# lvjiahui/DRT

Measured on AMD Instinct MI355X. Metric: M camera-rays/s (forward+backward) on 50k-tri mesh, 72 views, higher is better.
Workload: dtype f32 traversal + f64 shading/gradients; 1 GPU; horse_vh.ply x4 (1 midpoint subdivision) = 50248 tris / 25126 verts, 72 turntable views, 1024x1024 rays/view, LBVH rebuilt every step, forward+ray_loss+backward+all-reduce+SGD; targets=horse_scan.ply, mode=dropin, hip_graph=False, outputs_recycled=True, ray_binding=True, views_per_gpu=72, views_per_call=72

## Files before the change

### drt_amd/csrc/drt_api.hip

```cpp
#include "drt_scene.h"

static thread_local char g_err[512] = "";
int fail(int code, const char* fmt, ...) {
    va_list ap;
    va_start(ap, fmt);
    vsnprintf(g_err, sizeof(g_err), fmt, ap);
    va_end(ap);
    return code;
}

int ensure_slow_stack(drt_scene* s, hipStream_t st) {
    if (s->slow_stack) return DRT_OK;
    hipStreamCaptureStatus cap = hipStreamCaptureStatusNone;
    if (hipStreamIsCapturing(st, &cap) == hipSuccess && cap != hipStreamCaptureStatusNone)
        return fail(DRT_E_INVALID, "the first silhouette / closest-point / intersect query of a scene allocates its overflow area and cannot run inside a "
                                   "stream capture: issue one such call eagerly before capturing");
    int blocks = s->grid_trace;
    if (blocks < 4 * s->n_cu) blocks = 4 * s->n_cu;
    if (blocks < kRedoGrid) blocks = kRedoGrid;
    HIP_TRY(hipMalloc(&s->slow_stack, sizeof(int32_t) * (size_t)blocks * kTraceBlock * kStackSlowDev));
    return DRT_OK;
}

static int g_det = -1;
// ... 80 lines not shown
}

int drt_create(int device, drt_scene_t** out) {
    if (!out) return fail(DRT_E_INVALID, "out is null");
    int count = 0;
    HIP_TRY(hipGetDeviceCount(&count));
    if (device < 0 || device >= count) return fail(DRT_E_INVALID, "device %d out of range (%d visible)", device, count);
    HIP_TRY(hipSetDevice(device));
    drt_scene* s = new (std::nothrow) drt_scene();
    if (!s) return fail(DRT_E_NOMEM, "host allocation failed");
    s->device = device;
    hipError_t e = hipMalloc(&s->params, sizeof(BuildParams));
    if (e == hipSuccess) e = hipMalloc(&s->scratch, sizeof(unsigned long long) * 8);
    if (e == hipSuccess) e = hipMalloc(&s->bounds_acc, sizeof(uint32_t) * 12);
    if (e == hipSuccess) {
        const uint32_t init[12] = {0xFF800000u, 0xFF800000u, 0xFF800000u, 0x007FFFFFu, 0x007FFFFFu, 0x007FFFFFu,
                                   0xFF800000u, 0xFF800000u, 0xFF800000u, 0x007FFFFFu, 0x007FFFFFu, 0x007FFFFFu};
        e = hipMemcpy(s->bounds_acc, init, sizeof(init), hipMemcpyHostToDevice);
    }
    if (e == hipSuccess) e = hipMalloc(&s->vcount, sizeof(unsigned) * 4);
    if (e == hipSuccess) e = hipMemset(s->vcount, 0, sizeof(unsigned) * 4);
    if (e == hipSuccess) e = hipMalloc(&s->seg_counts, sizeof(unsigned) * drt_scene::kMaxSeg);
    if (e == hipSuccess) e = hipEventCreateWithFlags(&s->fork_ev, hipEventDisableTiming);
    if (e == hipSuccess) e = hipStreamCreateWithFlags(&s->build_stream, hipStreamNonBlocking);
    if (e == hipSuccess) e = hipEventCreateWithFlags(&s->prefill_fork, hipEventDisableTiming);
    if (e == hipSuccess) e = hipEventCreateWithFlags(&s->prefill_done, hipEventDisableTiming);
    if (e == hipSuccess) e = hipEventCreateWithFlags(&s->prefill_done_cap, hipEventDisableTiming);
    if (e == hipSuccess) e = hipEventCreateWithFlags(&s->build_fork, hipEventDisableTiming);
    if (e == hipSuccess) e = hipEventCreateWithFlags(&s->build_done, hipEventDisableTiming);
    if (const char* ev = getenv("DRT_ASYNC_BUILD")) s->async_build = atoi(ev) != 0;
    if (const char* ev = getenv("DRT_CULL_DIRECT")) s->cull_direct = atoi(ev) != 0;
    if (const char* ev = getenv("DRT_CULL_PARK")) s->cull_park = atoi(ev) != 0;
    if (const char* ev = getenv("DRT_CULL_DIRECT_MIN_LOG2")) { const int v = atoi(ev); if (v >= 0 && v <= 40) s->cull_direct_min_rays = (int64_t)1 << v; }
    if (const char* ev = getenv("DRT_TREE")) { const int v = atoi(ev); if (v >= 0 && v <= 2) s->tree_mode = v; }
    if (const char* ev = getenv("DRT_REBUILD_EVERY")) { const int v = atoi(ev); if (v >= 1) s->rebuild_every = v; }
    if (const char* ev = getenv("DRT_STREAMS")) { const int v = atoi(ev); if (v >= 1 && v <= drt_scene::kMaxSub) s->n_sub = v; }
    if (const char* ev = getenv("DRT_RASTER")) s->use_raster = atoi(ev) != 0;
    if (const char* ev = getenv("DRT_RASTER_DEAL")) s->raster_deal = atoi(ev) != 0;
    if (const char* ev = getenv("DRT_RASTER_DEAL_MIN_RUNS")) { const long long v = atoll(ev); if (v >= 0) s->raster_deal_min_runs = v; }
    if (const char* ev = getenv("DRT_RASTER_DEAL_FIXED")) { const int v = atoi(ev); if (v >= 1 && v <= 65536) s->raster_deal_fixed = (uint32_t)v; }
    if (const char* ev = getenv("DRT_HIT_SEED")) s->hit_seed = atoi(ev) != 0;
    if (const char* ev = getenv("DRT_ARM_FINISH_BESIDE")) s->arm_finish_beside = atoi(ev) != 0;
    if (const char* ev = getenv("DRT_SEED_TILED")) s->seed_tiled = atoi(ev) != 0;
    if (const char* ev = getenv("DRT_GRID_CANARY")) s->grid_canary = atoi(ev) != 0;
    if (const char* ev = getenv("DRT_FILL_OVERLAP")) s->fill_overlap = atoi(ev) != 0;
    if (const char* ev = getenv("DRT_FILL_AFTER_SHADE1")) s->fill_after_shade1 = atoi(ev) != 0;
    if (const char* ev = getenv("DRT_SUB_PER_STREAM")) { const int v = atoi(ev); if (v >= 1 && v <= 16) s->sub_per_stream = v; }
    if (const char* ev = getenv("DRT_MIN_SUB_LOG2")) { const int v = atoi(ev); if (v >= 12 && v <= 30) s->min_sub_rays = (int64_t)1 << v; }
    for (int k = 0; k < s->n_sub && e == hipSuccess; ++k) {
        drt_scene::Sub& w = s->sub[k];
        e = hipStreamCreateWithFlags(&w.stream, hipStreamNonBlocking);
        if (e == hipSuccess) e = hipEventCreateWithFlags(&w.done, hipEventDisableTiming);
        if (e == hipSuccess) e = hipEventCreateWithFlags(&w.tail, hipEventDisableTiming);
        if (e == hipSuccess) e = hipEventCreateWithFlags(&w.fill_fork, hipEventDisableTiming);
        if (e == hipSuccess) e = hipEventCreateWithFlags(&w.fill_join, hipEventDisableTiming);
        if (e == hipSuccess) e = hipMalloc(&w.qcount, sizeof(unsigned) * kQCount);
        if (e == hipSuccess) e = hipMalloc(&w.slow_stack, sizeof(int32_t) * (size_t)kRedoGrid * kTraceBlock * kStackSlowDev);
    }
    if (e == hipSuccess) {
        hipDeviceProp_t prop;
        if (hipGetDeviceProperties(&prop, device) == hipSuccess && prop.multiProcessorCount > 0) s->n_cu = prop.multiProcessorCount;
        int per_cu;
        per_cu = query_blocks_per_cu();
        s->grid_trace = s->n_cu * per_cu;
        if (s->grid_trace > kTraceGridMax) s->grid_trace = kTraceGridMax;
        per_cu = pipeline_blocks_per_cu();
        s->grid_path = s->n_cu * per_cu;
        if (s->grid_path * 2 > kTraceGridMax) s->grid_path = kTraceGridMax / 2;
        per_cu = mega_blocks_per_cu();
        s->grid_mega = s->n_cu * per_cu;
        if (const char* e = getenv("DRT_MEGA_BPC")) { const int v = atoi(e); if (v >= 1 && v <= 8) s->grid_mega = v * s->n_cu; }
        if (const char* e = getenv("DRT_MEGA_MAX_LOG2")) { const int v = atoi(e); s->mega_max_rays = v <= 0 ? 0 : (v <= 31 ? (int64_t)1 << v : (int64_t)1 << 31); }
        if (const char* e = getenv("DRT_SHADE_MIN")) { const int v = atoi(e); if (v >= 1 && v <= 64) s->shade_min = v; }
        if (const char* e = getenv("DRT_MEGA_REFILL_MIN")) { const int v = atoi(e); if (v >= 1 && v <= 64) s->mega_refill_min = v; }
        if (const char* e = getenv("DRT_TRACE_BPC")) { const int v = atoi(e); if (v >= 1 && v * s->n_cu * 2 <= kTraceGridMax) s->grid_path = v * s->n_cu; }
        if (const char* e = getenv("DRT_INNER_MIN")) { const int v = atoi(e); if (v >= 1 && v <= 64) s->inner_min = v; }
        if (const char* e = getenv("DRT_REFILL_MIN")) { const int v = atoi(e); if (v >= 1 && v <= 64) s->refill_min = v; }
        if (const char* e = getenv("DRT_CHUNK_LOG2")) { const int v = atoi(e); if (v >= 16 && v <= 30) s->chunk_rays = (int64_t)1 << v; }
    }
    if (e != hipSuccess) {
        drt_destroy(s);
        return fail(DRT_E_HIP, "hipMalloc: %s", hipGetErrorString(e));
    }
    *out = s;
    return DRT_OK;
}

void drt_destroy(drt_scene_t* s) {
    if (!s) return;
    (void)hipSetDevice(s->device);
    if (s->build_stream) (void)hipStreamSynchronize(s->build_stream);
    scene_free_mesh(s);
    if (s->build_fork) (void)hipEventDestroy(s->build_fork);
    if (s->build_done) (void)hipEventDestroy(s->build_done);
    if (s->build_stream) (void)hipStreamDestroy(s->build_stream);
    (void)hipFree(s->params);
    (void)hipFree(s->slow_stack);
    (void)hipFree(s->scratch); (void)hipFree(s->bounds_acc); (void)hipFree(s->seg_counts);
    (void)hipFree(s->b1_list); (void)hipFree(s->b1_redo); (void)hipFree(s->b1_count);
    for (int j = 0; j < drt_scene::kMaxSub; ++j) {
        drt_scene::Sub& w = s->sub[j];
        for (int k = 0; k < 3; ++k) { (void)hipFree(w.q_idx[k]); (void)hipFree(w.q_ray[k]); (void)hipFree(w.q_face[k]); }
        (void)hipFree(w.tmp_face1); (void)hipFree(w.tmp_face2); (void)hipFree(w.qcount); (void)hipFree(w.slow_stack); (void)hipFree(w.redo);
        (void)hipFree(w.zbuf); (void)hipFree(w.zmask); (void)hipFree(w.vmodel); (void)hipFree(w.big); (void)hipFree(w.big_count); (void)hipFree(w.gen_list); (void)hipFree(w.ray64);
        (void)hipFree(w.deal.table);
        if (w.done) (void)hipEventDestroy(w.done);
        if (w.fill_fork) (void)hipEventDestroy(w.fill_fork);
        if (w.fill_join) (void)hipEventDestroy(w.fill_join);
        if (w.tail) (void)hipEventDestroy(w.tail);
        if (w.stream) (void)hipStreamDestroy(w.stream);
    }
    image_views_free(s);
    image_loss_free(s);
    paths_free(s);
    (void)hipFree(s->vcount);
    (void)hipFree(s->vh_list);
    if (s->fork_ev) (void)hipEventDestroy(s->fork_ev);
    if (s->prefill_fork) (void)hipEventDestroy(s->prefill_fork);
    if (s->prefill_done) (void)hipEventDestroy(s->prefill_done);
    if (s->prefill_done_cap) (void)hipEventDestroy(s->prefill_done_cap);
    for (auto& e : s->prof_ev) (void)hipEventDestroy(e);
    (void)hipFree(s->prof_counts);
    delete s;
}

int drt_profile_enable(drt_scene_t* s, int on) {
    CHECK_SCENE(s);
    if (on && s->prof_ev.empty()) {
        s->prof_ev.resize(8192);
        s->prof_stage.resize(4096);
        for (auto& e : s->prof_ev) HIP_TRY(hipEventCreate(&e));
        HIP_TRY(hipMalloc(&s->prof_counts, sizeof(unsigned long long) * (kProfStages + 12)));
        HIP_TRY(hipMemset(s->prof_counts, 0, sizeof(unsigned long long) * (kProfStages + 12)));
    }
    s->prof_on = on != 0;
    s->prof_stats = on == 2;
    s->prof_serial = on == 3;
    return DRT_OK;
}

int drt_profile_select(drt_scene_t* s, uint32_t stage_mask) {
// ... 77 lines not shown
```

### drt_amd/csrc/drt_pipeline.hip

```cpp
#include "drt_device.h"
#include "drt_trace_kernel.h"
#include "drt_pathsink.h"


struct Ray64 {
    double* o;
    double* d;
};
struct Pipe {
    RayList r0, r1, r2;
    unsigned* count;
    unsigned* valid;
    int32_t* redo;
};




__device__ __forceinline__ void write_dead(int64_t i, double* out_ori, double* out_dir, uint8_t* mask, int32_t* face2) {
    const d3 z{0.0, 0.0, 0.0};
    store_d3(out_ori, i, z);
    store_d3(out_dir, i, z);
    mask[3 * i] = 0; mask[3 * i + 1] = 0; mask[3 * i + 2] = 0;
    face2[i] = -1;
// ... 1098 lines not shown
        w.tmp_face1 = w.tmp_face2 = nullptr; w.fused_cap = 0;
        HIP_TRY(hipMalloc(&w.tmp_face1, sizeof(int32_t) * n));
        HIP_TRY(hipMalloc(&w.tmp_face2, sizeof(int32_t) * n));
        w.fused_cap = n;
    }
    return DRT_OK;
}

static Pipe pipe_of(const drt_scene* s, const drt_scene::Sub& w) {
    return Pipe{RayList{w.q_idx[0], w.q_ray[0], w.q_face[0]}, RayList{w.q_idx[1], w.q_ray[1], w.q_face[1]},
                RayList{w.q_idx[2], w.q_ray[2], w.q_face[2]}, w.qcount, s->vcount, w.redo};
}

struct Plan { int64_t size; int count; int streams; };
static Plan plan_call(const drt_scene* s, int64_t n_rays, int tile_w, int tile_h) {
    int64_t unit = 256;
    if (tile_w >= 64 && tile_w % 64 == 0) unit = 4 * (int64_t)tile_w;
    if (unit > 256 && tile_h >= 4 && tile_h % 4 == 0 && n_rays % ((int64_t)tile_w * tile_h) == 0) unit = (int64_t)tile_w * tile_h;
    int64_t count = (n_rays + s->chunk_rays - 1) / s->chunk_rays;
    const int64_t by_min = n_rays / s->min_sub_rays;
    const int64_t most = (int64_t)s->n_sub * s->sub_per_stream;
    const int64_t want = by_min < most ? by_min : most;
    if (want > count) count = want;
    if (count < 1) count = 1;
    int64_t size = (n_rays + count - 1) / count;
    size = (size + unit - 1) / unit * unit;
    count = (n_rays + size - 1) / size;
    Plan pl;
    pl.size = size; pl.count = (int)count; pl.streams = count < s->n_sub ? (int)count : s->n_sub;
    if (s->prof_serial) pl.streams = 1;
    return pl;
}

__global__ void k_store_models(const ViewModel* __restrict__ work, ViewModel* __restrict__ cache, int n) {
    const int v = blockIdx.x * blockDim.x + threadIdx.x;
    if (v >= n) return;
    ViewModel m = work[v];
    m.all = (m.ok && m.all) ? 1 : 0;
    m.ok = m.all;
    cache[v] = m;
}

static bool raster_on(const drt_scene* s, int64_t n, int tile_w, int tile_h) {
    if (!s->use_raster || s->n_faces <= 0 || tile_w < 64 || tile_w % 64 != 0 || tile_h < 4 || tile_h % 4 != 0) return false;
    const int64_t image = (int64_t)tile_w * tile_h;
    return n > 0 && n % image == 0 && n / image <= 65535;
}

constexpr int kIntPreOri = 1 << 16, kIntPreDir = 1 << 17, kIntPreMask = 1 << 18, kIntMask = kIntPreOri | kIntPreDir | kIntPreMask;
extern "C++" {
template <bool FUSED>
static int launch_chunk(drt_scene* s, drt_scene::Sub& w, hipStream_t st, const PathCtx& pc, const Pipe& p, const double* o, const double* d, const uint8_t* valid,
                        int64_t n, double* out_ori, double* out_dir, uint8_t* mask, int32_t* face1, int32_t* face2, int tile_w, int tile_h,
                        int grid_mode, ViewModel* grid_cache ,
                        hipStream_t aux , int64_t chunk_base, int32_t* valid_idx,
                        bool* n_finished ,
                        int32_t* seed2 = nullptr ) {
    if (n_finished) *n_finished = false;
    const bool sparse_faces = (grid_mode & DRT_GRID_SPARSE_FACES) != 0;
    const bool pre_ori = (grid_mode & kIntPreOri) != 0, pre_dir = (grid_mode & kIntPreDir) != 0, pre_mask = (grid_mode & kIntPreMask) != 0;
    const bool all_verified = (grid_mode & DRT_GRID_ALL_VERIFIED) != 0 && (grid_mode & 3) == DRT_GRID_TRUST && grid_cache;
    grid_mode &= 3;
    const int gs = 8 * s->n_cu;
    if (tile_w < 64 || tile_w % 64 != 0 || n % (4 * (int64_t)tile_w) != 0) tile_w = 0;
    RasterIn rz{nullptr, 0, nullptr, nullptr, nullptr, 0, 0, 0, 0};
    const bool mega = s->mega_max_rays > 0 && n <= s->mega_max_rays && n_finished != nullptr;
    const Ray64 r64 = !mega ? Ray64{nullptr, nullptr} : (FUSED ? Ray64{w.ray64, w.ray64 + 3 * n} : Ray64{out_ori, out_dir});
    bool late_fill = false;
    hipStream_t fs = s->prof_serial ? st : s->build_stream;
    {
        hipStreamCaptureStatus cs = hipStreamCaptureStatusNone;
        if (fs != st && hipStreamIsCapturing(st, &cs) == hipSuccess && cs != hipStreamCaptureStatusNone) fs = aux ? aux : st;
    }
    const int64_t image = (int64_t)tile_w * tile_h;
    if (raster_on(s, n, tile_w, tile_h)) {
        const int n_views = (int)(n / image);
        int rc = ensure_raster(s, w, n, n_views, st);
        if (rc) return rc;
        if (!grid_cache) grid_mode = DRT_GRID_NONE;
        if (!FUSED && grid_mode == DRT_GRID_TRUST) {
            late_fill = s->fill_overlap;
            if (!late_fill) {
                StageTimer t(s, st, kStageFill);
                if (!pre_ori) (void)hipMemsetAsync(out_ori, 0, sizeof(double) * 3 * n, st);
                if (!pre_dir) (void)hipMemsetAsync(out_dir, 0, sizeof(double) * 3 * n, st);
                if (!pre_mask) (void)hipMemsetAsync(mask, 0, 3 * n, st);
            }
            if (!sparse_faces) { (void)hipMemsetAsync(face1, 0xFF, sizeof(int32_t) * n, st); (void)hipMemsetAsync(face2, 0xFF, sizeof(int32_t) * n, st); }
        }
        if (late_fill && mega) {
            if (fs != st && aux) fs = aux;
            if (fs != st) { HIP_TRY(hipEventRecord(w.fill_fork, st)); HIP_TRY(hipStreamWaitEvent(fs, w.fill_fork, 0)); }
            { StageTimer tf(s, fs, kStageFill);
              if (!pre_ori) (void)hipMemsetAsync(out_ori, 0, sizeof(double) * 3 * n, fs);
              if (!pre_dir) (void)hipMemsetAsync(out_dir, 0, sizeof(double) * 3 * n, fs);
              if (!pre_mask) (void)hipMemsetAsync(mask, 0, 3 * n, fs); }
            if (fs != st) HIP_TRY(hipEventRecord(w.fill_join, fs));
        }
        StageTimer t(s, st, kStageRaster);
        rc = launch_raster(s, w, st, o, d, n_views, tile_w, tile_h, grid_mode == DRT_GRID_TRUST ? grid_cache : nullptr);
        if (rc) return rc;
        rz = RasterIn{w.vmodel, grid_mode, w.zbuf, w.zmask, w.gen_list, tile_w, tile_h, all_verified ? 1 : 0, all_verified ? 1 : 0};
    }
    const bool pre_any = pre_ori || pre_dir || pre_mask;
    if (pre_any && !late_fill) HIP_TRY(hipStreamWaitEvent(st, s->prefill_done, 0));
    const bool tree_late = all_verified && rz.views != nullptr;
    if (!tree_late) { int rc = wait_build(s, st); if (rc) return rc; }
    const bool direct = s->cull_direct && rz.views && grid_mode == DRT_GRID_TRUST && !mega && n >= s->cull_direct_min_rays;
    const bool park = !FUSED && !mega && rz.views && grid_mode == DRT_GRID_TRUST && pre_ori && pre_dir && pre_mask && s->cull_park;
    const Ray64 r64p = park ? Ray64{out_ori, out_dir} : r64;
    if (park) HIP_TRY(hipStreamWaitEvent(st, s->prefill_done, 0));
    {
        int64_t* rc = s->route_counts;
        rc[kRouteTotal] += 1;
        rc[kRouteRaster] += rz.views != nullptr;
        rc[kRouteTrust] += rz.views && grid_mode == DRT_GRID_TRUST;
        rc[kRouteDirect] += direct;
        rc[kRoutePark] += park;
        rc[kRouteLateFill] += late_fill;
        rc[kRouteTreeLate] += tree_late;
        rc[kRouteMega] += mega;
    }
    { StageTimer t(s, st, kStageCull);
      const unsigned n_patches = (unsigned)((n + kPathBlock - 1) / kPathBlock);
      if (rz.views && grid_mode == DRT_GRID_TRUST) {
          uint32_t* list = reinterpret_cast<uint32_t*>(p.redo);
          k_patch_list<<<(n_patches + kPathBlock - 1) / kPathBlock, kPathBlock, 0, st>>>(n_patches, tile_w, rz, list, p.count + 7);
          static const int cull_per_cu = cull_blocks_per_cu();
          const unsigned few = (unsigned)(kCullFewPerCu * s->n_cu), long_list = few * (unsigned)(kCullRun * kCullLongRuns);
          k_cull_listed<FUSED><<<cull_per_cu * s->n_cu, kPathBlock, 0, st>>>(list, p.count + 7, pc.tc.nodes, pc.tc.n_tris, o, d, valid, n, out_ori, out_dir, mask, face1, face2, p, tile_w, rz,
                                                          pc, direct, late_fill, park ? Ray64{out_ori, out_dir} : Ray64{nullptr, nullptr}, few, long_list);
      } else {
          k_cull<FUSED><<<n_patches, kPathBlock, 0, st>>>(pc.tc.nodes, pc.tc.n_tris, o, d, valid, n, out_ori, out_dir, mask, face1, face2, p, tile_w, rz,
                                                          pre_ori && pre_dir && pre_mask && sparse_faces);
      } }
    auto issue_late_fills = [&]() -> int {
        if (fs != st) { HIP_TRY(hipEventRecord(w.fill_fork, st)); HIP_TRY(hipStreamWaitEvent(fs, w.fill_fork, 0)); }
        { StageTimer tf(s, fs, kStageFill);
          if (!pre_ori) (void)hipMemsetAsync(out_ori, 0, sizeof(double) * 3 * n, fs);
          if (!pre_dir) (void)hipMemsetAsync(out_dir, 0, sizeof(double) * 3 * n, fs);
          if (!pre_mask) (void)hipMemsetAsync(mask, 0, 3 * n, fs); }
        if (fs != st) HIP_TRY(hipEventRecord(w.fill_join, fs));
        return DRT_OK;
    };
    const bool fills_after_shade1 = s->fill_after_shade1 && fs != st;
    if (late_fill && !mega && !fills_after_shade1) { int rc = issue_late_fills(); if (rc) return rc; }
    if (rz.views && grid_mode == DRT_GRID_ESTABLISH)
        k_store_models<<<(int)(n / ((int64_t)tile_w * tile_h) + 63) / 64, 64, 0, st>>>(w.vmodel, grid_cache, (int)(n / ((int64_t)tile_w * tile_h)));
    { StageTimer t(s, st, kStageTrace1);
      if (rz.views && all_verified) {
      } else if (rz.views) {
          const TraceOut out{p.r0.face, nullptr, nullptr, w.gen_list};
          launch_trace_list(kTraceClosestListed, s->grid_path, st, pc.tc, p.r0.ray, p.count + 3, out, p.redo, p.count + 4, p.count + 16, s->refill_min, s->inner_min, s->prof_stats ? s->prof_counts + kProfStages + 4 * 0 : nullptr);
      } else {
          launch_trace_list(kTraceClosest, s->grid_path, st, pc.tc, p.r0.ray, p.count + 0, TraceOut{p.r0.face, nullptr, nullptr, nullptr}, p.redo, p.count + 4, p.count + 16, s->refill_min, s->inner_min, s->prof_stats ? s->prof_counts + kProfStages + 4 * 0 : nullptr);
      } }
    if (mega) {
        if (late_fill && fs != st) HIP_TRY(hipStreamWaitEvent(st, w.fill_join, 0));
        if (pre_any) HIP_TRY(hipStreamWaitEvent(st, s->prefill_done, 0));
    }
    {
      StageTimer t(s, st, kStageShade1);
// ... 138 lines not shown
    for (int k = 0; k < pl.streams; ++k) { int rc = ensure_queues(s->sub[k], pl.size, false); if (rc) return rc; }
    HIP_TRY(hipMemsetAsync(s->vcount, 0, sizeof(unsigned), st));
    const bool segmented = d_valid_idx != nullptr && pl.count >= 2 && pl.count <= drt_scene::kMaxSeg;
    if (segmented) HIP_TRY(hipMemsetAsync(s->seg_counts, 0, sizeof(unsigned) * pl.count, st));
    s->segs = drt_scene::Segs{};
    grid_mode &= ~kIntMask;
    hipStreamCaptureStatus cap = hipStreamCaptureStatusNone;
    (void)hipStreamIsCapturing(st, &cap);
    if (arm.loss && (cap != hipStreamCaptureStatusNone || (s->mega_max_rays > 0 && n_rays - (pl.count - 1) * pl.size <= s->mega_max_rays)))
        arm = drt_scene::LossArm{};
    if (s->n_prefill && (cap == hipStreamCaptureStatusNone || (s->clean.rows && s->clean.captured))) {
        int matched = 0;
        for (int k = 0; k < s->n_prefill; ++k) {
            const drt_scene::Prefill& f = s->prefill[k];
            const int before = grid_mode;
            if (f.ptr == d_out_ori && f.bytes == (int64_t)sizeof(double) * 3 * n_rays) grid_mode |= kIntPreOri;
            if (f.ptr == d_out_dir && f.bytes == (int64_t)sizeof(double) * 3 * n_rays) grid_mode |= kIntPreDir;
            if (f.ptr == d_mask && f.bytes == 3 * n_rays) grid_mode |= kIntPreMask;
            matched += grid_mode != before;
        }
        if (matched != s->n_prefill && cap == hipStreamCaptureStatusNone) HIP_TRY(hipStreamWaitEvent(st, s->prefill_done, 0));
        s->n_prefill = 0;
    }
    bool clean_late = s->clean.rows != nullptr && (grid_mode & 3) == DRT_GRID_TRUST && d_grid_cache != nullptr;
    for (int j = 0; j < pl.count && clean_late; ++j) {
        const int64_t b = j * pl.size, n = n_rays - b < pl.size ? n_rays - b : pl.size;
        clean_late = raster_on(s, n, tile_w, tile_h);
    }
    int rc = DRT_OK;
    if (s->clean.rows && !clean_late) { rc = flush_clean(s, st); if (rc) return rc; }
    rc = fork_streams(s, st, pl.streams);
    if (rc) return rc;
    if (s->clean.rows) { rc = flush_clean(s, st); if (rc) return rc; }
    bool finish_moved = false;
    for (int j = 0; j < pl.count; ++j) {
        drt_scene::Sub& w = s->sub[j % pl.streams];
        const int64_t b = j * pl.size;
        const int64_t n = n_rays - b < pl.size ? n_rays - b : pl.size;
        const PathCtx pc = sub_ctx(s, w, d_verts, ior_int, ior_ext);
        Pipe p = pipe_of(s, w);
        int32_t* vlist = d_valid_idx;
        if (segmented) { p.valid = s->seg_counts + j; vlist = d_valid_idx + b; }
        HIP_TRY(hipMemsetAsync(w.qcount, 0, kQCount * sizeof(unsigned), w.stream));
        bool finished = false;
        rc = launch_chunk<false>(s, w, w.stream, pc, p, d_origin + 3 * b, d_dir + 3 * b, nullptr, n, d_out_ori + 3 * b, d_out_dir + 3 * b,
                                 d_mask + 3 * b, d_face1 + b, d_face2 + b, tile_w, tile_h, grid_mode, sub_cache(d_grid_cache, b, tile_w, tile_h),
                                 st, b, vlist, &finished, seed2 ? seed2 + b : nullptr);
        if (rc) return rc;
        if (!finished) {
            hipStream_t fin = w.stream;
            if (arm.loss && s->arm_finish_beside && !s->prof_serial && j + pl.streams >= pl.count) {
                HIP_TRY(hipEventRecord(w.tail, w.stream));
                HIP_TRY(hipStreamWaitEvent(st, w.tail, 0));
                fin = st;
                finish_moved = true;
            }
            StageTimer t(s, fin, kStageFinish);
            k_finish<<<8 * s->n_cu, kPathBlock, 0, fin>>>(d_out_ori + 3 * b, d_out_dir + 3 * b, d_mask + 3 * b, d_face2 + b, p, b, vlist);
        }
        if (arm.loss) {
            if (finished) return fail(DRT_E_INVALID, "armed loss: a sub-batch took the one-kernel path");
            StageTimer t(s, w.stream, kStageBackward);
            DET_LAUNCH(k_loss_bwd_armed, DRT_BWD_BPC * s->n_cu, 256, w.stream, pc, d_origin + 3 * b, d_dir + 3 * b, arm.screen_pixel + 3 * b, arm.valid + b,
                                                                 d_face1 + b, d_face2 + b, p, arm.loss, arm.grad_verts);
        }
        if (s->prof_on) k_prof_counts<<<1, 64, 0, w.stream>>>(w.qcount, (unsigned long long)n, s->prof_counts, 0, raster_on(s, n, tile_w, tile_h), finished);
    }
    rc = join_streams(s, st, pl.streams);
    if (rc) return rc;
    if (segmented) {
        for (int j = 1; j < pl.count; ++j)
            k_join_lists<<<2 * s->n_cu, 256, 0, st>>>(d_valid_idx, s->seg_counts, j, (int64_t)j * pl.size, j + 1 == pl.count, s->vcount, d_n_valid);
        if (cap == hipStreamCaptureStatusNone && !finish_moved) s->segs = drt_scene::Segs{d_valid_idx, pl.count, 0};
    } else if (d_n_valid) {
        k_store_count<<<1, 64, 0, st>>>(s->vcount, d_n_valid);
    }
    if (s->prof_on) s->prof_stream = st;
    HIP_TRY(hipGetLastError());
    s->loss_taken = arm.loss != nullptr;
    return DRT_OK;
// ... 232 lines not shown
    HIP_TRY(hipGetLastError());
    return DRT_OK;
}

int drt_scale_rows3(double* d_x, const int32_t* d_list, const uint32_t* d_n_list, const double* d_scale, void* stream) {
    if (!d_x || !d_list || !d_n_list || !d_scale) return fail(DRT_E_INVALID, "null pointer argument");
    k_scale_rows3<<<1024, 256, 0, (hipStream_t)stream>>>(d_x, d_list, d_n_list, d_scale);
    HIP_TRY(hipGetLastError());
    return DRT_OK;
}

int drt_render_ray_loss_fused(drt_scene_t* s, const double* d_verts, const double* d_origin, const double* d_dir,
                              const double* d_screen_pixel, const uint8_t* d_valid, int64_t n_rays, double ior_int,
                              double ior_ext, double* d_loss, double* d_grad_verts, int64_t* d_n_valid, int tile_w, int tile_h,
                              int grid_mode, void* d_grid_cache, void* stream) {
    CHECK_BUILT(s);
    if (n_rays < 0 || n_rays > INT32_MAX) return fail(DRT_E_INVALID, "ray count out of range");
    if (n_rays == 0) return DRT_OK;
    if (!d_verts || !d_origin || !d_dir || !d_screen_pixel || !d_valid || !d_loss || !d_grad_verts) return fail(DRT_E_INVALID, "null pointer argument");
    hipStream_t st = (hipStream_t)stream;
    int32_t* const seed2 = take_seed(s, n_rays);
    (void)take_loss_arm(s, -1);
    const Plan pl = plan_call(s, n_rays, tile_w, tile_h);
    for (int k = 0; k < pl.streams; ++k) { int rc = ensure_queues(s->sub[k], pl.size, true, s->mega_max_rays > 0 && pl.size <= s->mega_max_rays); if (rc) return rc; }
    hipStreamCaptureStatus cap = hipStreamCaptureStatusNone;
    (void)hipStreamIsCapturing(st, &cap);
    if (s->n_prefill && cap == hipStreamCaptureStatusNone) {
        HIP_TRY(hipStreamWaitEvent(st, s->prefill_done, 0));
        s->n_prefill = 0;
    }
    int rc = fork_streams(s, st, pl.streams);
    if (rc) return rc;
    grid_mode &= ~kIntMask;
    for (int j = 0; j < pl.count; ++j) {
        drt_scene::Sub& w = s->sub[j % pl.streams];
        const int64_t b = j * pl.size;
        const int64_t n = n_rays - b < pl.size ? n_rays - b : pl.size;
        const PathCtx pc = sub_ctx(s, w, d_verts, ior_int, ior_ext);
        const Pipe p = pipe_of(s, w);
        HIP_TRY(hipMemsetAsync(w.qcount, 0, kQCount * sizeof(unsigned), w.stream));
        bool finished = false;
        rc = launch_chunk<true>(s, w, w.stream, pc, p, d_origin + 3 * b, d_dir + 3 * b, d_valid + b, n, nullptr, nullptr, nullptr, w.tmp_face1, w.tmp_face2, tile_w, tile_h, grid_mode, sub_cache(d_grid_cache, b, tile_w, tile_h),
                                st, b, nullptr, &finished, seed2 ? seed2 + b : nullptr);
        if (rc) return rc;
        { StageTimer t(s, w.stream, kStageLossBwdFused);
          DET_LAUNCH(k_loss_bwd_fused, DRT_BWD_BPC * s->n_cu, 256, w.stream, pc, d_origin + 3 * b, d_dir + 3 * b, d_screen_pixel + 3 * b, w.tmp_face1, w.tmp_face2, p,
                                                               d_loss, d_grad_verts, reinterpret_cast<unsigned long long*>(d_n_valid)); }
        if (s->prof_on) k_prof_counts<<<1, 64, 0, w.stream>>>(w.qcount, (unsigned long long)n, s->prof_counts, 1, raster_on(s, n, tile_w, tile_h), finished);
    }
    rc = join_streams(s, st, pl.streams);
    if (rc) return rc;
    if (s->prof_on) s->prof_stream = st;
    HIP_TRY(hipGetLastError());
    return DRT_OK;
}


}
```

### drt_amd/csrc/drt_raster.hip

```cpp
#include "drt_device.h"

__global__ void __launch_bounds__(64) k_fit_views(const double* __restrict__ origin, const double* __restrict__ dir, int w, int h,
                                                  ViewModel* __restrict__ views) {
    __shared__ ViewModel vm;
    const int64_t base = (int64_t)blockIdx.x * w * h;
    if (threadIdx.x == 0) {
        const int64_t i00 = base, iW0 = base + (w - 1), i0H = base + (int64_t)(h - 1) * w, iWH = i0H + (w - 1);
        if (fit_view_model(load_d3(origin, i00), load_d3(dir, i00), load_d3(dir, iW0), load_d3(dir, i0H), load_d3(dir, iWH),
                           (double)(w - 1), (double)(h - 1), vm))
            vm.ok = 1;
    }
    __syncthreads();
    bool good = vm.ok != 0;
    if (good) {
        const int sx = (int)(threadIdx.x & 7), sy = (int)(threadIdx.x >> 3);
        const int x = (int)(((int64_t)(w - 1) * sx) / 7), y = (int)(((int64_t)(h - 1) * sy) / 7);
        const int64_t i = base + (int64_t)y * w + x;
        good = view_verify(vm, load_d3(origin, i), load_d3(dir, i), (double)x, (double)y);
    }
    const bool all_good = __ballot(good) == ~0ull;
    if (threadIdx.x == 0) {
        vm.ok = all_good ? 1 : 0;
        vm.all = vm.ok;
        views[blockIdx.x] = vm;
// ... 236 lines not shown
constexpr int64_t kRasterDealMaxRuns = (int64_t)1 << 18;
static int64_t raster_runs(int64_t n_tris, int n_views) { return (n_tris + 63) / 64 * n_views; }

int ensure_raster(drt_scene* s, drt_scene::Sub& w, int64_t n_rays, int n_views, hipStream_t st) {
    if (n_rays > w.z_cap) {
        (void)hipFree(w.zbuf); (void)hipFree(w.zmask);
        w.zbuf = nullptr; w.zmask = nullptr; w.z_cap = 0;
        const int64_t words = (n_rays + 2047) / 2048 + 1;
        HIP_TRY(hipMalloc(&w.zbuf, sizeof(unsigned long long) * n_rays));
        HIP_TRY(hipMalloc(&w.zmask, sizeof(uint32_t) * words));
        k_fill_u64<<<4 * s->n_cu, 256, 0, st>>>(w.zbuf, n_rays, kRasterEmpty);
        HIP_TRY(hipMemsetAsync(w.zmask, 0, sizeof(uint32_t) * words, st));
        w.z_cap = n_rays;
    }
    if (n_views > w.vm_cap) {
        (void)hipFree(w.vmodel); w.vmodel = nullptr; w.vm_cap = 0;
        HIP_TRY(hipMalloc(&w.vmodel, sizeof(ViewModel) * n_views));
        w.vm_cap = n_views;
    }
    if (!w.big) HIP_TRY(hipMalloc(&w.big, sizeof(BigItem) * drt_scene::kBigCap));
    drt_scene::Sub::Deal& dl = w.deal;
    if (!w.big_count) {
        const int n_waves = 8 * s->n_cu * 4;
        HIP_TRY(hipMalloc(&w.big_count, sizeof(unsigned) * (kRasterCostAt + (s->raster_deal ? 2 * kRasterDealMaxRuns : 0))));
        if (s->raster_deal) {
            HIP_TRY(hipMalloc(&dl.table, sizeof(DealPos) * 2 * (n_waves + 1)));
            dl.cap_runs = kRasterDealMaxRuns; dl.cap_waves = n_waves;
        }
    }
    return DRT_OK;
}

int launch_raster(drt_scene* s, drt_scene::Sub& w, hipStream_t st, const double* d_origin, const double* d_dir, int n_views, int iw, int ih,
                  ViewModel* trusted) {
    const int n = (int)s->n_faces;
    HIP_TRY(hipMemsetAsync(w.big_count, 0, sizeof(unsigned), st));
    if (trusted) k_check_views<<<n_views, 64, 0, st>>>(d_origin, d_dir, iw, ih, trusted, w.vmodel,
                                                        s->grid_canary ? (++s->canary_salt ? s->canary_salt : ++s->canary_salt) : 0u,
                                                        s->vcount + 3);
    else k_fit_views<<<n_views, 64, 0, st>>>(d_origin, d_dir, iw, ih, w.vmodel);
    if (n > 0) {
        drt_scene::Sub::Deal& dl = w.deal;
        const int grid = 8 * s->n_cu;
        const int64_t n_runs = raster_runs(n, n_views);
        const bool record = s->raster_deal && dl.table && n_runs > 0 && n_runs >= s->raster_deal_min_runs && n_runs <= dl.cap_runs && grid * 4 == dl.cap_waves;
        const bool dealt = record && dl.complete && dl.dir == d_dir && dl.n_views == n_views && dl.iw == iw && dl.ih == ih && dl.n_tris == n && dl.grid == grid;
        s->raster_deal_counts[dealt ? 0 : 1] += 2;
        for (int pass = 0; pass < 2; ++pass) {
            auto* const kern = pass == 0 ? (dealt ? k_raster<true, true, 0> : record ? k_raster<false, true, 0> : k_raster<false, false, 0>)
                                         : (dealt ? k_raster<true, true, 1> : record ? k_raster<false, true, 1> : k_raster<false, false, 1>);
            kern<<<grid, 256, 0, st>>>(s->tris_flat, n, w.vmodel, n_views, d_dir, iw, ih, w.zbuf, w.zmask, reinterpret_cast<BigItem*>(w.big), w.big_count,
                                       dealt ? dl.table + pass * (dl.cap_waves + 1) : nullptr);
            if (pass == 0) {
                k_raster_big<<<8 * s->n_cu, 256, 0, st>>>(s->tris_flat, w.vmodel, d_dir, iw, ih, w.zbuf, w.zmask,
                                                           reinterpret_cast<const BigItem*>(w.big), w.big_count, drt_scene::kBigCap);
                HIP_TRY(hipMemsetAsync(w.big_count, 0, sizeof(unsigned), st));
            }
        }
        k_raster_big<<<8 * s->n_cu, 256, 0, st>>>(s->tris_flat, w.vmodel, d_dir, iw, ih, w.zbuf, w.zmask,
                                                   reinterpret_cast<const BigItem*>(w.big), w.big_count, drt_scene::kBigCap);
        dl.complete = false;
        if (record) {
            k_raster_deal<<<dim3((unsigned)((n_runs + kDealBlock - 1) / kDealBlock), 2), kDealBlock, 0, st>>>(w.big_count, dl.table, (unsigned)n_runs, (unsigned)(grid * 4), s->raster_deal_fixed);
            dl.dir = d_dir; dl.n_views = n_views; dl.iw = iw; dl.ih = ih; dl.n_tris = n; dl.grid = grid;
            dl.complete = true;
        }
    }
    HIP_TRY(hipGetLastError());
    return DRT_OK;
}
```

### drt_amd/csrc/drt_scene.h

```cpp
#pragma once
#include <hip/hip_runtime.h>

#include <cstdarg>
#include <cstdio>
#include <cstdlib>
#include <cstring>
#include <new>
#include <vector>

#include "../../include/drt_hip.h"
#include "drt_common.h"
#include "drt_closest.h"
#include "drt_edge.h"
#include "drt_fixed.h"
#include "drt_lbvh.h"
#include "drt_path.h"
#include "drt_raster.h"
#include "drt_shade.h"
#include "drt_traverse.h"
#include "drt_tri.h"

using namespace drt;


// ... 24 lines not shown
static_assert(kProfStages == DRT_PROFILE_STAGES, "include/drt_hip.h");

struct BuildParams {
    float lox, loy, loz;
    float ix, iy, iz;
    float pad;
    int32_t reserved;
    MortonPlan plan;
};

struct drt_scene {
    int device = 0;
    int64_t n_faces = 0, n_verts = 0;
    int64_t cap_faces = 0, cap_verts = 0;
    int32_t* faces = nullptr;
    float* verts = nullptr;
    Node* nodes = nullptr;
    Node4Q* wide = nullptr;
    int32_t *range_lo = nullptr, *range_hi = nullptr;
    TriRec* tris = nullptr;
    TriRec* tris_flat = nullptr;
    int32_t* slot_of_face = nullptr;
    struct Seed { int32_t* face2 = nullptr; int64_t n = 0; } seed;
    struct LossArm { const double* screen_pixel = nullptr; const uint8_t* valid = nullptr; double* loss = nullptr; double* grad_verts = nullptr; int64_t n = 0; } loss_arm;
    bool loss_taken = false;
    hipStream_t build_stream = nullptr;
    hipEvent_t build_fork = nullptr, build_done = nullptr;
    bool build_pending = false;
    bool order_valid = false;
    int sorted_buf = 0;
    bool cull_direct = true;
    bool cull_park = true;
    int64_t cull_direct_min_rays = (int64_t)1 << 25;
    int64_t route_counts[8] = {0};
    int tree_mode = 0, rebuild_every = 1, since_full = 0;
    bool topology_fixed = false;
    uint32_t* bounds_acc = nullptr;
    bool async_build = true;
    uint32_t *keys[2] = {nullptr, nullptr}, *idx[2] = {nullptr, nullptr};
    uint32_t* hist = nullptr;
    int32_t *parent_inner = nullptr, *parent_leaf = nullptr;
    uint32_t* flags = nullptr;
    BuildParams* params = nullptr;
    int32_t* slow_stack = nullptr;
    unsigned long long* scratch = nullptr;
    int32_t *b1_list = nullptr, *b1_redo = nullptr;
    unsigned* b1_count = nullptr;
    int64_t b1_cap = 0;
    struct Sub {
        hipStream_t stream = nullptr;
        hipEvent_t done = nullptr;
        hipEvent_t tail = nullptr;
        hipEvent_t fill_fork = nullptr, fill_join = nullptr;
        int32_t* q_idx[3] = {nullptr, nullptr, nullptr};
        float* q_ray[3] = {nullptr, nullptr, nullptr};
        int32_t* q_face[3] = {nullptr, nullptr, nullptr};
        int32_t *tmp_face1 = nullptr, *tmp_face2 = nullptr;
        unsigned* qcount = nullptr;
        double* ray64 = nullptr;
        int64_t ray64_cap = 0;
        int32_t* redo = nullptr;
        int32_t* slow_stack = nullptr;
        int64_t q_cap = 0, fused_cap = 0;
        unsigned long long* zbuf = nullptr;
        uint32_t* zmask = nullptr;
        int64_t z_cap = 0;
        ViewModel* vmodel = nullptr;
        int vm_cap = 0;
        void* big = nullptr;
        unsigned* big_count = nullptr;
        int32_t* gen_list = nullptr;
        struct Deal {
            DealPos* table = nullptr;
            int64_t cap_runs = 0;
            int cap_waves = 0;
            const double* dir = nullptr;
            int n_views = 0, iw = 0, ih = 0, n_tris = 0, grid = 0;
            bool complete = false;
        } deal;
    };
    static constexpr unsigned kBigCap = 1u << 20;
    static constexpr int kMaxSub = 4;
    Sub sub[kMaxSub];
    int n_sub = 2;
    int sub_per_stream = 1;
    int64_t min_sub_rays = 1 << 24;
// ... 13 lines not shown
    bool prof_on = false;
    uint32_t prof_mask = ~0u;
    bool prof_stats = false;
    bool prof_serial = false;
    std::vector<hipEvent_t> prof_ev;
    std::vector<int> prof_stage;
    size_t prof_used = 0;
    size_t prof_dropped = 0;
    unsigned long long* prof_counts = nullptr;
    hipStream_t prof_stream = nullptr;
    int n_cu = 256;
    int grid_trace = 2048;
    int grid_path = 2048;
    int64_t trace_stats[12] = {0};
    int grid_mega = 1024;
    int64_t mega_max_rays = 0;
    int shade_min = 8;
    int mega_refill_min = 16;
    int refill_min = 32;
    int inner_min = 24;
    int64_t chunk_rays = kChunkRays;

    bool fill_after_shade1 = true;
    bool fill_overlap = true;
    bool grid_canary = true;
    unsigned canary_salt = 0;
    bool seed_tiled = true;
    bool arm_finish_beside = true;
    bool hit_seed = true;
    bool use_raster = true;
    bool raster_deal = true;
    int64_t raster_deal_min_runs = 16384;
    uint32_t raster_deal_fixed = kRasterDealFixed;
    int64_t raster_deal_counts[2] = {0, 0};
    bool built = false;
    void* paths_ws = nullptr;
    void* image_loss_ws = nullptr;
    void* image_views = nullptr;
};


int query_blocks_per_cu();
int pipeline_blocks_per_cu();
int mega_blocks_per_cu();

int ensure_raster(drt_scene* s, drt_scene::Sub& w, int64_t n_rays, int n_views, hipStream_t st);
int launch_raster(drt_scene* s, drt_scene::Sub& w, hipStream_t st, const double* d_origin, const double* d_dir, int n_views, int iw, int ih,
                  ViewModel* trusted);

void paths_free(drt_scene* s);
void image_loss_free(drt_scene* s);
void image_views_free(drt_scene* s);

int ensure_slow_stack(drt_scene* s, hipStream_t st);
bool det_mode();
#define DET_LAUNCH(kern, grid, block, st, ...)                                        \
    do {                                                                              \
        if (det_mode()) kern<true><<<grid, block, 0, st>>>(__VA_ARGS__);              \
        else kern<false><<<grid, block, 0, st>>>(__VA_ARGS__);                        \
    } while (0)
int check_counters_pipeline(unsigned long long* out4);
int check_counters_trace(unsigned long long* out4);

void scene_free_mesh(drt_scene* s);
int ensure_capacity(drt_scene* s, int64_t n_faces, int64_t n_verts);
int rebuild(drt_scene* s, hipStream_t st, const uint32_t* acc);
int wait_build(drt_scene* s, hipStream_t st);

inline int grid_for(int64_t n, int block, int cap) {
    int64_t g = (n + block - 1) / block;
    if (g < 1) g = 1;
    if (g > cap) g = cap;
    return (int)g;
}

inline TraceCtx trace_ctx(const drt_scene* s) { return TraceCtx{s->wide, s->tris, (int)s->n_faces, s->slow_stack}; }
inline PathCtx path_ctx(const drt_scene* s, const double* d_verts, double ior_int, double ior_ext) {
    return PathCtx{trace_ctx(s), s->faces, d_verts, ior_int, ior_ext};
}

#define CHECK_SCENE(s)                                                        \
// ... 42 lines not shown
```

Measured before the change: 46760 M camera-rays/s.

## Launch raster deal kernel on aux stream beside chunk; tune head-chunk cull few threshold

Splits the raster deal kernel out of launch_raster so it can be issued on the auxiliary stream (forked by event) when there are no more chunks than streams, letting it overlap with the subsequent work on the chunk stream. Also makes the cull 'few' threshold for the first chunk configurable, defaulting to 2 per CU instead of the fixed constant. The beside launch risks races if downstream consumers of the deal table on the chunk stream are not joined back to the aux stream.

After: 46560 M camera-rays/s. Within noise of the previous version (-0.4%).

```diff
diff --git a/drt_amd/csrc/drt_api.hip b/drt_amd/csrc/drt_api.hip
--- a/drt_amd/csrc/drt_api.hip
+++ b/drt_amd/csrc/drt_api.hip
@@ -136,6 +136,8 @@
     if (const char* ev = getenv("DRT_CULL_DIRECT")) s->cull_direct = atoi(ev) != 0;
     if (const char* ev = getenv("DRT_CULL_PARK")) s->cull_park = atoi(ev) != 0;
     if (const char* ev = getenv("DRT_CULL_DIRECT_MIN_LOG2")) { const int v = atoi(ev); if (v >= 0 && v <= 40) s->cull_direct_min_rays = (int64_t)1 << v; }
+    if (const char* ev = getenv("DRT_CULL_HEAD_PER_CU")) { const int v = atoi(ev); if (v >= 1 && v <= 8) s->cull_head_per_cu = v; }
+    if (const char* ev = getenv("DRT_RASTER_DEAL_BESIDE")) s->raster_deal_beside = atoi(ev) != 0;
     if (const char* ev = getenv("DRT_TREE")) { const int v = atoi(ev); if (v >= 0 && v <= 2) s->tree_mode = v; }
     if (const char* ev = getenv("DRT_REBUILD_EVERY")) { const int v = atoi(ev); if (v >= 1) s->rebuild_every = v; }
     if (const char* ev = getenv("DRT_STREAMS")) { const int v = atoi(ev); if (v >= 1 && v <= drt_scene::kMaxSub) s->n_sub = v; }
@@ -158,6 +160,7 @@
         if (e == hipSuccess) e = hipEventCreateWithFlags(&w.tail, hipEventDisableTiming);
         if (e == hipSuccess) e = hipEventCreateWithFlags(&w.fill_fork, hipEventDisableTiming);
         if (e == hipSuccess) e = hipEventCreateWithFlags(&w.fill_join, hipEventDisableTiming);
+        if (e == hipSuccess) e = hipEventCreateWithFlags(&w.deal_fork, hipEventDisableTiming);
         if (e == hipSuccess) e = hipMalloc(&w.qcount, sizeof(unsigned) * kQCount);
         if (e == hipSuccess) e = hipMalloc(&w.slow_stack, sizeof(int32_t) * (size_t)kRedoGrid * kTraceBlock * kStackSlowDev);
     }
@@ -211,6 +214,7 @@
         if (w.done) (void)hipEventDestroy(w.done);
         if (w.fill_fork) (void)hipEventDestroy(w.fill_fork);
         if (w.fill_join) (void)hipEventDestroy(w.fill_join);
+        if (w.deal_fork) (void)hipEventDestroy(w.deal_fork);
         if (w.tail) (void)hipEventDestroy(w.tail);
         if (w.stream) (void)hipStreamDestroy(w.stream);
     }
diff --git a/drt_amd/csrc/drt_pipeline.hip b/drt_amd/csrc/drt_pipeline.hip
--- a/drt_amd/csrc/drt_pipeline.hip
+++ b/drt_amd/csrc/drt_pipeline.hip
@@ -1154,6 +1154,8 @@
     return pl;
 }
 
+static bool deal_goes_beside(const drt_scene* s, const Plan& pl) { return s->raster_deal_beside && !s->prof_serial && pl.count <= pl.streams; }
+
 __global__ void k_store_models(const ViewModel* __restrict__ work, ViewModel* __restrict__ cache, int n) {
     const int v = blockIdx.x * blockDim.x + threadIdx.x;
     if (v >= n) return;
@@ -1177,7 +1179,8 @@
                         int grid_mode, ViewModel* grid_cache ,
                         hipStream_t aux , int64_t chunk_base, int32_t* valid_idx,
                         bool* n_finished ,
-                        int32_t* seed2 = nullptr ) {
+                        int32_t* seed2 = nullptr ,
+                        bool deal_beside = false ) {
     if (n_finished) *n_finished = false;
     const bool sparse_faces = (grid_mode & DRT_GRID_SPARSE_FACES) != 0;
     const bool pre_ori = (grid_mode & kIntPreOri) != 0, pre_dir = (grid_mode & kIntPreDir) != 0, pre_mask = (grid_mode & kIntPreMask) != 0;
@@ -1220,8 +1223,10 @@
             if (fs != st) HIP_TRY(hipEventRecord(w.fill_join, fs));
         }
         StageTimer t(s, st, kStageRaster);
-        rc = launch_raster(s, w, st, o, d, n_views, tile_w, tile_h, grid_mode == DRT_GRID_TRUST ? grid_cache : nullptr);
+        bool deal_due = false;
+        rc = launch_raster(s, w, st, o, d, n_views, tile_w, tile_h, grid_mode == DRT_GRID_TRUST ? grid_cache : nullptr, &deal_due);
         if (rc) return rc;
+        if (deal_due) { rc = launch_raster_deal(s, w, st, deal_beside ? aux : st); if (rc) return rc; }
         rz = RasterIn{w.vmodel, grid_mode, w.zbuf, w.zmask, w.gen_list, tile_w, tile_h, all_verified ? 1 : 0, all_verified ? 1 : 0};
     }
     const bool pre_any = pre_ori || pre_dir || pre_mask;
@@ -1249,7 +1254,8 @@
           uint32_t* list = reinterpret_cast<uint32_t*>(p.redo);
           k_patch_list<<<(n_patches + kPathBlock - 1) / kPathBlock, kPathBlock, 0, st>>>(n_patches, tile_w, rz, list, p.count + 7);
           static const int cull_per_cu = cull_blocks_per_cu();
-          const unsigned few = (unsigned)(kCullFewPerCu * s->n_cu), long_list = few * (unsigned)(kCullRun * kCullLongRuns);
+          const unsigned few = (unsigned)((chunk_base == 0 ? s->cull_head_per_cu : kCullFewPerCu) * s->n_cu);
+          const unsigned long_list = (unsigned)(kCullFewPerCu * s->n_cu) * (unsigned)(kCullRun * kCullLongRuns);
           k_cull_listed<FUSED><<<cull_per_cu * s->n_cu, kPathBlock, 0, st>>>(list, p.count + 7, pc.tc.nodes, pc.tc.n_tris, o, d, valid, n, out_ori, out_dir, mask, face1, face2, p, tile_w, rz,
                                                           pc, direct, late_fill, park ? Ray64{out_ori, out_dir} : Ray64{nullptr, nullptr}, few, long_list);
       } else {
@@ -1454,6 +1460,7 @@
     rc = fork_streams(s, st, pl.streams);
     if (rc) return rc;
     if (s->clean.rows) { rc = flush_clean(s, st); if (rc) return rc; }
+    const bool deal_beside = deal_goes_beside(s, pl);
     bool finish_moved = false;
     for (int j = 0; j < pl.count; ++j) {
         drt_scene::Sub& w = s->sub[j % pl.streams];
@@ -1467,7 +1474,7 @@
         bool finished = false;
         rc = launch_chunk<false>(s, w, w.stream, pc, p, d_origin + 3 * b, d_dir + 3 * b, nullptr, n, d_out_ori + 3 * b, d_out_dir + 3 * b,
                                  d_mask + 3 * b, d_face1 + b, d_face2 + b, tile_w, tile_h, grid_mode, sub_cache(d_grid_cache, b, tile_w, tile_h),
-                                 st, b, vlist, &finished, seed2 ? seed2 + b : nullptr);
+                                 st, b, vlist, &finished, seed2 ? seed2 + b : nullptr, deal_beside);
         if (rc) return rc;
         if (!finished) {
             hipStream_t fin = w.stream;
@@ -1766,6 +1773,7 @@
     int rc = fork_streams(s, st, pl.streams);
     if (rc) return rc;
     grid_mode &= ~kIntMask;
+    const bool deal_beside = deal_goes_beside(s, pl);
     for (int j = 0; j < pl.count; ++j) {
         drt_scene::Sub& w = s->sub[j % pl.streams];
         const int64_t b = j * pl.size;
@@ -1775,7 +1783,7 @@
         HIP_TRY(hipMemsetAsync(w.qcount, 0, kQCount * sizeof(unsigned), w.stream));
         bool finished = false;
         rc = launch_chunk<true>(s, w, w.stream, pc, p, d_origin + 3 * b, d_dir + 3 * b, d_valid + b, n, nullptr, nullptr, nullptr, w.tmp_face1, w.tmp_face2, tile_w, tile_h, grid_mode, sub_cache(d_grid_cache, b, tile_w, tile_h),
-                                st, b, nullptr, &finished, seed2 ? seed2 + b : nullptr);
+                                st, b, nullptr, &finished, seed2 ? seed2 + b : nullptr, deal_beside);
         if (rc) return rc;
         { StageTimer t(s, w.stream, kStageLossBwdFused);
           DET_LAUNCH(k_loss_bwd_fused, DRT_BWD_BPC * s->n_cu, 256, w.stream, pc, d_origin + 3 * b, d_dir + 3 * b, d_screen_pixel + 3 * b, w.tmp_face1, w.tmp_face2, p,
diff --git a/drt_amd/csrc/drt_raster.hip b/drt_amd/csrc/drt_raster.hip
--- a/drt_amd/csrc/drt_raster.hip
+++ b/drt_amd/csrc/drt_raster.hip
@@ -292,8 +292,9 @@
 }
 
 int launch_raster(drt_scene* s, drt_scene::Sub& w, hipStream_t st, const double* d_origin, const double* d_dir, int n_views, int iw, int ih,
-                  ViewModel* trusted) {
+                  ViewModel* trusted, bool* deal_due ) {
     const int n = (int)s->n_faces;
+    *deal_due = false;
     HIP_TRY(hipMemsetAsync(w.big_count, 0, sizeof(unsigned), st));
     if (trusted) k_check_views<<<n_views, 64, 0, st>>>(d_origin, d_dir, iw, ih, trusted, w.vmodel,
                                                         s->grid_canary ? (++s->canary_salt ? s->canary_salt : ++s->canary_salt) : 0u,
@@ -321,11 +322,23 @@
                                                    reinterpret_cast<const BigItem*>(w.big), w.big_count, drt_scene::kBigCap);
         dl.complete = false;
         if (record) {
-            k_raster_deal<<<dim3((unsigned)((n_runs + kDealBlock - 1) / kDealBlock), 2), kDealBlock, 0, st>>>(w.big_count, dl.table, (unsigned)n_runs, (unsigned)(grid * 4), s->raster_deal_fixed);
             dl.dir = d_dir; dl.n_views = n_views; dl.iw = iw; dl.ih = ih; dl.n_tris = n; dl.grid = grid;
-            dl.complete = true;
+            *deal_due = true;
         }
     }
     HIP_TRY(hipGetLastError());
     return DRT_OK;
 }
+
+int launch_raster_deal(drt_scene* s, drt_scene::Sub& w, hipStream_t st, hipStream_t on) {
+    drt_scene::Sub::Deal& dl = w.deal;
+    const int64_t n_runs = raster_runs(dl.n_tris, dl.n_views);
+    if (on != st) {
+        HIP_TRY(hipEventRecord(w.deal_fork, st));
+        HIP_TRY(hipStreamWaitEvent(on, w.deal_fork, 0));
+    }
+    k_raster_deal<<<dim3((unsigned)((n_runs + kDealBlock - 1) / kDealBlock), 2), kDealBlock, 0, on>>>(w.big_count, dl.table, (unsigned)n_runs, (unsigned)(dl.grid * 4), s->raster_deal_fixed);
+    dl.complete = true;
+    HIP_TRY(hipGetLastError());
+    return DRT_OK;
+}
diff --git a/drt_amd/csrc/drt_scene.h b/drt_amd/csrc/drt_scene.h
--- a/drt_amd/csrc/drt_scene.h
+++ b/drt_amd/csrc/drt_scene.h
@@ -80,6 +80,7 @@
     bool cull_direct = true;
     bool cull_park = true;
     int64_t cull_direct_min_rays = (int64_t)1 << 25;
+    int cull_head_per_cu = 2;
     int64_t route_counts[8] = {0};
     int tree_mode = 0, rebuild_every = 1, since_full = 0;
     bool topology_fixed = false;
@@ -100,6 +101,7 @@
         hipEvent_t done = nullptr;
         hipEvent_t tail = nullptr;
         hipEvent_t fill_fork = nullptr, fill_join = nullptr;
+        hipEvent_t deal_fork = nullptr;
         int32_t* q_idx[3] = {nullptr, nullptr, nullptr};
         float* q_ray[3] = {nullptr, nullptr, nullptr};
         int32_t* q_face[3] = {nullptr, nullptr, nullptr};
@@ -179,6 +181,7 @@
     bool raster_deal = true;
     int64_t raster_deal_min_runs = 16384;
     uint32_t raster_deal_fixed = kRasterDealFixed;
+    bool raster_deal_beside = true;
     int64_t raster_deal_counts[2] = {0, 0};
     bool built = false;
     void* paths_ws = nullptr;
@@ -193,7 +196,8 @@
 
 int ensure_raster(drt_scene* s, drt_scene::Sub& w, int64_t n_rays, int n_views, hipStream_t st);
 int launch_raster(drt_scene* s, drt_scene::Sub& w, hipStream_t st, const double* d_origin, const double* d_dir, int n_views, int iw, int ih,
-                  ViewModel* trusted);
+                  ViewModel* trusted, bool* deal_due);
+int launch_raster_deal(drt_scene* s, drt_scene::Sub& w, hipStream_t st, hipStream_t on);
 
 void paths_free(drt_scene* s);
 void image_loss_free(drt_scene* s);
```
